# tvlabs/edge264

Measured on AMD Instinct MI355X. Metric: 1080p frames/s/GPU (bit-exact YUV) + achieved HBM GB/s vs 8 TB/s peak, higher is better.
Workload: dtype u8

## Files before the change

### edge264_amd/csrc/e264_intra.h

```cpp
#ifndef E264_INTRA_H
#define E264_INTRA_H
#include "e264_dev.h"

namespace {
#ifndef E264_HOST_INTRINSICS
E264_DEV uint32_t v_sad_u8(uint32_t a, uint32_t b, uint32_t c) { return __builtin_amdgcn_sad_u8(a, b, c); }
E264_DEV int relane(int lane) { asm volatile("" : "+v"(lane)); return lane; }
#endif

#define YT_STRIDE 32
#define YT(y, x) ytile[((y) + 1) * YT_STRIDE + (x) + 8]
#define CT_STRIDE 16
#define CT(p, y, x) ctile[p][((y) + 1) * CT_STRIDE + (x) + 4]

#define T4_STRIDE 20
struct __attribute__((aligned(16))) WaveLds {
	int16_t res[384];
	int32_t tmp[16 * T4_STRIDE];
	int32_t dc[24];
	uint8_t ytile[17 * YT_STRIDE];
	uint8_t ctile[2][9 * CT_STRIDE];
	__attribute__((aligned(4))) uint8_t fz[32];
	uint8_t pad_[8];
	__attribute__((aligned(4))) uint8_t lcol[3][16];
// ... 111 lines not shown
	int16_t *t16 = (int16_t *)L.tmp;
	if (on) {
		const int nb = __builtin_popcount(coded & 0x1111u & ((1u << (b * 4)) - 1));
		int div = qP / 6, m = qP - div * 6;
		const int shl = max(div - 6, 0), shr = max(6 - div, 0), rnd = div < 6 ? 1 << (5 - div) : 0;
		const int lo = div < 6 ? -32768 : (int)0x80000000, hi = div < 6 ? 32767 : 0x7fffffff;
		int16_t d[8];
		int lev[8];
		if (l8) {
#pragma unroll
			for (int i = 0; i < 8; i++) lev[i] = ((const int8_t *)coef_base)[nb * 64 + i * 8 + j];
		} else {
#pragma unroll
			for (int i = 0; i < 8; i++) lev[i] = ((const int16_t *)coef_base)[nb * 64 + i * 8 + j];
		}
#pragma unroll
		for (int i = 0; i < 8; i++) {
			int pos = i * 8 + j;
			int LS = wS[pos] * norm8(m, pos);
			d[i] = (int16_t)min(max((mul24(lev[i], (int)(int16_t)(LS << shl)) + rnd) >> shr, lo), hi);
		}
		idct8_1d(d);
#pragma unroll
		for (int i = 0; i < 8; i++)
			t16[b * 64 + i * 8 + j] = d[i];
	}
	wave_sync();
	if (on) {
		int i = j;
		int16_t d[8];
#pragma unroll
		for (int jj = 0; jj < 8; jj++)
			d[jj] = t16[b * 64 + i * 8 + jj];
		d[0] = (int16_t)(d[0] + 32);
		idct8_1d(d);
		int16_t *r = L.res + BYf(b * 4) * 16 + BXf(b * 4) + i;
#pragma unroll
		for (int jj = 0; jj < 8; jj++)
			r[jj * 16] = (int16_t)(d[jj] >> 6);
	}
	wave_sync();
}

E264_DEV int coef_dwords(const MbInfo &m)
{
	if (m.kind == E264_MB_ABSENT || m.kind == E264_MB_PCM || m.coded == 0)
		return 0;
	const uint32_t c = m.coded;
	int ac = __builtin_popcount(c >> 16 & 0xff) * 32;
	ac += (m.kind != E264_MB_I16x16 && (m.flags & E264_MBF_T8x8)) ? __builtin_popcount(c & 0x1111) * 128 : __builtin_popcount(c & 0xffff) * 32;
	if (m.flags & E264_MBF_LEV8) ac >>= 1;
	return (((c & E264_CODED_LUMA_DC) ? 32 : 0) + ((c & E264_CODED_CHROMA_DC) ? 16 : 0) + ac + 3) >> 2;
}
E264_DEV void coef_dma(int16_t *dst, const FrameCtx &f, const MbInfo &m, int lane)
{
	const int ndw = coef_dwords(m);
	if (ndw == 0)
		return;
	const gu32 *src = (const gu32 *)(f.payload + m.payload_off) + lane;
#ifndef E264_HOST_INTRINSICS
	typedef __attribute__((address_space(3))) void *lds_p;
	if (lane < ndw) __builtin_amdgcn_global_load_lds(src, (lds_p)dst, 4, 0, 0);
	if (ndw > 64 && 64 + lane < ndw) __builtin_amdgcn_global_load_lds(src + 64, (lds_p)(dst + 128), 4, 0, 0);
	if (ndw > 128 && 128 + lane < ndw) __builtin_amdgcn_global_load_lds(src + 128, (lds_p)(dst + 256), 4, 0, 0);
	if (ndw > 192 && 192 + lane < ndw) __builtin_amdgcn_global_load_lds(src + 192, (lds_p)(dst + 384), 4, 0, 0);
#else
	for (int k = 0; k < 4; k++)
		if (64 * k + lane < ndw) ((uint32_t *)dst)[64 * k + lane] = src[64 * k];
#endif
}
E264_DEV void coef_dma_wait()
{
#ifndef E264_HOST_INTRINSICS
	asm volatile("s_waitcnt vmcnt(0)" ::: "memory");
#endif
	wave_sync();
}
E264_DEV void slice_cache(WaveLds &L, const FrameCtx &f, int slice, int lane)
{
	if (E264_FIRST(L.ws_slice) == slice)
		return;
	cslice_t s = f.slices + slice;
	wave_sync();
	const gu32 *g4 = (const gu32 *)((const gu8 *)s + offsetof(E264SliceParams, weightScale4x4));
	const gu32 *g8 = (const gu32 *)((const gu8 *)s + offsetof(E264SliceParams, weightScale8x8));
	if (lane < 24) ((uint32_t *)L.ws)[lane] = g4[lane];
	else if (lane < 56) ((uint32_t *)L.ws)[lane] = g8[lane - 24];
	if (lane == 0) { L.ws_slice = slice; L.ws_idc = s->weighted_bipred_idc; }
	wave_sync();
}

template <int PLANES = 3>
E264_DEV void compute_residual(WaveLds &L, const int16_t *coefs, const FrameCtx &f, const MbInfo &m, bool inter, int lane)
{
	uint32_t *rz = (uint32_t *)L.res;
	rz[lane] = 0; rz[lane + 64] = 0; rz[lane + 128] = 0;
	const uint32_t coded = m.coded;
	const int16_t *pl = coefs;
	const int16_t *ldc = nullptr, *cdc = nullptr;
	if (coded & E264_CODED_LUMA_DC) { ldc = pl; pl += 16; }
	if (coded & E264_CODED_CHROMA_DC) { cdc = pl; pl += 8; }
	const uint8_t *co = (const uint8_t *)pl;
	const bool l8 = m.flags & E264_MBF_LEV8;
	const int lsz = l8 ? 1 : 2;
	const uint8_t *ws4 = L.ws, *ws8 = L.ws + 96;
	if (lane < 24) L.dc[lane] = 0;
	wave_sync();
	if (!coded) return;

	if ((PLANES & 1) && ldc && lane < 16) {
		int r = lane >> 2, l = lane & 3, acc = 0;
#pragma unroll
		for (int i = 0; i < 4; i++)
#pragma unroll
			for (int mm = 0; mm < 4; mm++) {
				int v = ldc[4 * i + mm];
				bool neg = (((0xA6C0 >> (4 * r)) >> mm) ^ ((0xA6C0 >> (4 * l)) >> i)) & 1;
				acc += neg ? -v : v;
			}
		int qP = m.qp[0];
		int LS = (ws4[0] * norm4(qP % 6, 0)) << (qP / 6);
		int k = (r >> 1) * 8 + (l >> 1) * 4 + (r & 1) * 2 + (l & 1);
		L.dc[k] = (int)((uint32_t)acc * (uint32_t)LS + 32u) >> 6;
	}
	if ((PLANES & 2) && cdc && lane >= 16 && lane < 24) {
		int n = lane & 3, pc = (lane >> 2) & 1;
		int c0 = cdc[pc], c4 = cdc[4 + pc], c2 = cdc[2 + pc], c6 = cdc[6 + pc];
		int v = n == 0 ? c0 + c4 + c2 + c6 : n == 1 ? c0 - c4 + c2 - c6 : n == 2 ? c0 + c4 - c2 - c6 : c0 - c4 - c2 + c6;
		int qP = pc ? m.qp[2] : m.qp[1];
		int LS = (ws4[(1 + pc + (inter ? 3 : 0)) * 16] * norm4(qP % 6, 0)) << (qP / 6);
		L.dc[16 + pc * 4 + n] = (int)((uint32_t)v * (uint32_t)LS) >> 5;
	}
	wave_sync();

	if (m.kind == E264_MB_I16x16) {
		if ((PLANES & 1) && (coded & (0xffff | E264_CODED_LUMA_DC)))
			idct4x4_blocks(L, 16, coded & 0xffff, true, ldc != nullptr, co, l8, ws4, m.qp[0], 0, 0, 16, lane);
		co += __builtin_popcount(coded & 0xffff) * 16 * lsz;
	} else if (m.flags & E264_MBF_T8x8) {
		if ((PLANES & 1) && (coded & 0x1111))
			idct8x8_blocks(L, coded, co, l8, ws8 + (inter ? 64 : 0), m.qp[0], lane);
		co += __builtin_popcount(coded & 0x1111) * 64 * lsz;
	} else {
		if ((PLANES & 1) && (coded & 0xffff))
			idct4x4_blocks(L, 16, coded & 0xffff, false, false, co, l8, ws4 + (inter ? 3 : 0) * 16, m.qp[0], 0, 0, 16, lane);
		co += __builtin_popcount(coded & 0xffff) * 16 * lsz;
	}
	if ((PLANES & 2) && (coded & (0xff0000 | E264_CODED_CHROMA_DC))) {
		int k = lane >> 2;
		int pc = (k >> 2) & 1;
		idct4x4_blocks(L, 8, coded >> 16 & 0xff, true, cdc != nullptr, co, l8, ws4 + (1 + pc + (inter ? 3 : 0)) * 16, pc ? m.qp[2] : m.qp[1], 16, 256, 8, lane);
	}
}

#define LP(l, m, r) (((l) + 2 * (m) + (r) + 2) >> 2)
#ifndef E264_I4_UNROLL
#define E264_I4_UNROLL 10
#endif
#include "e264_intra_tab.h"

struct IntraNb { uint32_t y, c; bool oky, okc; };
E264_DEV IntraNb issue_intra_neighbours(const FrameCtx &f, int mbx, int mby, int lane)
{
	IntraNb n;
	const bool left = lane >= 32 && lane < 48;
	const bool topY = lane < 25;
	const int x = lane - 1, gx = mbx * 16 + x;
	n.oky = topY ? (mby > 0 && gx >= 0 && gx < f.W) : (left && mbx > 0);
	const gu8 *Y = f.cur + (size_t)(mby * 16) * f.sY + mbx * 16;
	const ptrdiff_t offY = topY ? (ptrdiff_t)x - f.sY : (ptrdiff_t)(lane - 32) * f.sY - 1;
	if (n.oky) n.y = Y[offY];
	const bool topC = lane < 18;
	const int xc = lane % 9 - 1;
	const int pl = topC ? lane / 9 : (lane - 32) >> 3;
	n.okc = topC ? (mby > 0 && mbx * 8 + xc >= 0) : (left && mbx > 0);
	const gu8 *C = plane_base(f, f.cur, 1 + (pl & 1)) + (size_t)(mby * 8) * f.sC + mbx * 8;
	const ptrdiff_t offC = topC ? (ptrdiff_t)xc - f.sC : (ptrdiff_t)(lane & 7) * f.sC - 1;
	if (n.okc) n.c = C[offC];
	return n;
}
E264_DEV void commit_intra_neighbours(WaveLds &L, const IntraNb &n, int lane)
{
	const bool left = lane >= 32 && lane < 48;
	const uint8_t vy = n.oky ? (uint8_t)n.y : 0, vc = n.okc ? (uint8_t)n.c : 0;
	if (lane < 25) L.YT(-1, lane - 1) = vy;
	else if (left) { L.YT(lane - 32, -1) = vy; L.lcol[0][lane - 32] = vy; }
	if (lane < 18) L.CT(lane / 9, -1, lane % 9 - 1) = vc;
	else if (left) { L.CT((lane - 32) >> 3, lane & 7, -1) = vc; L.lcol[1 + ((lane - 32) >> 3)][lane & 7] = vc; }
	wave_sync();
}

E264_DEV int intra4x4_tab(const WaveLds &L, uint32_t e, int X0, int Y0, int mode)
{
	const uint8_t *org = &L.YT(Y0 - 1, X0 - 1);
	const bool dc = mode >= 2 && mode <= 5;
	const int a = org[e & 255], b = org[e >> 8 & 255], c = org[e >> 16 & 255];
	int vd = 128;
	if (dc) {
		const uint32_t w = *(const uint32_t *)(org + 1);
		const int st = (int)v_sad_u8(w, 0, 0);
		const int sl = org[YT_STRIDE] + org[2 * YT_STRIDE] + org[3 * YT_STRIDE] + org[4 * YT_STRIDE];
		vd = mode == 2 ? (st + sl + 4) >> 3 : mode == 3 ? (st + 2) >> 2 : mode == 4 ? (sl + 2) >> 2 : 128;
	}
	const int ty = (int)(e >> 24), sh = ty >> 3;
	const int v = (a + (ty & 3) * b + ((ty & 4) ? c : 0) + ((1 << sh) >> 1)) >> sh;
	return dc ? vd : v;
}

E264_DEV int intra4x4_px(const WaveLds &L, int X0, int Y0, int mode, int x, int y)
{
#define T(i) ((int)L.YT(Y0 - 1, X0 + (i)))
#define Lf(i) ((int)L.YT(Y0 + (i), X0 - 1))
#define TR(i) ((i) < 4 || has_tr ? T(i) : T(3))
	const bool has_tr = (mode == 6 || mode == 11);
	switch (mode) {
	default:
	case 0: return T(x);
	case 1: return Lf(y);
	case 2: return (T(0) + T(1) + T(2) + T(3) + Lf(0) + Lf(1) + Lf(2) + Lf(3) + 4) >> 3;
	case 3: return (T(0) + T(1) + T(2) + T(3) + 2) >> 2;
	case 4: return (Lf(0) + Lf(1) + Lf(2) + Lf(3) + 2) >> 2;
	case 5: return 128;
	case 6: case 7:
		return (x == 3 && y == 3) ? (TR(6) + 3 * TR(7) + 2) >> 2 : LP(TR(x + y), TR(x + y + 1), TR(x + y + 2));
	case 8:
		if (x > y) return LP(T(x - y - 2), T(x - y - 1), T(x - y));
		if (x < y) return LP(y - x - 2 < 0 ? T(-1) : Lf(y - x - 2), Lf(y - x - 1), Lf(y - x));
		return LP(T(0), T(-1), Lf(0));
	case 9: {
		int z = 2 * x - y, i = x - (y >> 1);
		if (z >= 0 && !(z & 1)) return (T(i - 1) + T(i) + 1) >> 1;
		if (z >= 0) return LP(T(i - 2), T(i - 1), T(i));
		if (z == -1) return LP(Lf(0), T(-1), T(0));
		return LP(Lf(y - 1), Lf(y - 2), y - 3 < 0 ? T(-1) : Lf(y - 3)); }
	case 10: {
		int z = 2 * y - x, i = y - (x >> 1);
#define L_(j) ((j) < 0 ? T(-1) : Lf(j))
// ... 78 lines not shown
		const int corner = T(-1);
		int Hh = 0, V = 0;
		for (int i = 0; i < 8; i++) {
			Hh += (i + 1) * (byte_of(tw, 8 + i) - (i == 7 ? corner : byte_of(tw, 6 - i)));
			V += (i + 1) * (byte_of(lw, 8 + i) - (i == 7 ? corner : byte_of(lw, 6 - i)));
		}
		int a = 16 * (byte_of(lw, 15) + byte_of(tw, 15)), b = (5 * Hh + 32) >> 6, c = (5 * V + 32) >> 6;
		for (int i = 0; i < 4; i++) out[i] = clip255((a + b * (X + i - 7) + c * (Yr - 7) + 16) >> 5);
		return; }
	}
#undef T
#undef Lf
}

E264_DEV int intra_chroma_px(const WaveLds &L, int p, int mode, int x, int y)
{
#define T(i) ((int)L.CT(p, -1, (i)))
#define Lf(i) ((int)L.CT(p, (i), -1))
	switch (mode) {
	default:
	case 0: case 1: case 2: case 3: {
		if (mode == 3) return 128;
		int bx = x >> 2, by = y >> 2;
		int t = 0, l = 0;
		t = (int)v_sad_u8(*(const uint32_t *)&L.CT(p, -1, bx * 4), 0, 0);
		l = (int)v_sad_u8(((const uint32_t *)L.lcol[1 + p])[by], 0, 0);
		if (mode == 1) return (t + 2) >> 2;
		if (mode == 2) return (l + 2) >> 2;
		if (bx == by) return (t + l + 4) >> 3;
		return bx ? (t + 2) >> 2 : (l + 2) >> 2; }
	case 4: return Lf(y);
	case 5: return T(x);
	case 6: {
		const uint32_t tw[2] = {*(const uint32_t *)&L.CT(p, -1, 0), *(const uint32_t *)&L.CT(p, -1, 4)};
		const uint32_t lw[2] = {((const uint32_t *)L.lcol[1 + p])[0], ((const uint32_t *)L.lcol[1 + p])[1]};
		const int corner = T(-1);
		int Hh = 0, V = 0;
		for (int i = 0; i < 4; i++) {
			Hh += (i + 1) * (byte_of(tw, 4 + i) - (i == 3 ? corner : byte_of(tw, 2 - i)));
			V += (i + 1) * (byte_of(lw, 4 + i) - (i == 3 ? corner : byte_of(lw, 2 - i)));
		}
		int a = 16 * (byte_of(lw, 7) + byte_of(tw, 7)), b = (34 * Hh + 32) >> 6, c = (34 * V + 32) >> 6;
		return clip255((a + b * (x - 3) + c * (y - 3) + 16) >> 5); }
	}
#undef T
#undef Lf
}

#ifndef E264_INTRA_LAUNDER
#define E264_INTRA_LAUNDER 5
#endif
template <int WHICH, int PLANES = 3>
E264_DEV void recon_mb(WaveLds &L, const FrameCtx &f, const MbInfo &m, int mbx, int mby, int lane, const uint32_t *i4tab, const int16_t *coefs,
	int16_t *coefs_next, const uint32_t *next_rec, MbInfo &mn PH_PARAMS)
{
	if (m.kind == E264_MB_ABSENT)
		return;
	const bool par = m.kind == E264_MB_INTER || m.kind == E264_MB_PCM;
	if ((WHICH == 1 && !par) || (WHICH == 2 && par))
		return;
	cslice_t s = f.slices + m.slice;
	const gu8 *pl = f.payload + m.payload_off;
	const int k = lane >> 2, r = lane & 3;
	const int X = BXf(k), Yr = BYf(k) + r;
	gu8 *dY = f.cur + (size_t)(mby * 16 + Yr) * f.sY + mbx * 16 + X;
	const int cpl = lane >> 5, cy = (lane >> 2) & 7, cx = (lane & 3) * 2;
	gu8 *dC = plane_base(f, f.cur, 1 + cpl) + (size_t)(mby * 8 + cy) * f.sC + mbx * 8 + cx;

	if (m.kind == E264_MB_PCM) {
		*(gu32 *)dY = *(const gu32 *)(pl + Yr * 16 + X);
		*(gu16 *)dC = *(const gu16 *)(pl + 256 + cpl * 64 + cy * 8 + cx);
		return;
	}
	const uint32_t modes_lo = m.modes_lo, modes_hi = m.modes_hi;
	IntraNb nbv;
	nbv.oky = nbv.okc = false;
	if (WHICH != 1 && m.kind != E264_MB_INTER)
		nbv = issue_intra_neighbours(f, mbx, mby, (E264_INTRA_LAUNDER & 2) ? relane(lane) : lane);
	PH(2);
	if (next_rec) {
		mn = mb_from_lds(next_rec);
		coef_dma(coefs_next, f, mn, lane);
	}
	slice_cache(L, f, m.slice, lane);
	PH(3);
	compute_residual<PLANES>(L, coefs, f, m, WHICH == 2 ? false : m.kind == E264_MB_INTER, (E264_INTRA_LAUNDER & 4) ? relane(lane) : lane);
	PH(4);

	int pY[4], pC[2];
	bool tile_luma = false;
	if (WHICH != 1 && m.kind != E264_MB_INTER) {
		commit_intra_neighbours(L, nbv, (E264_INTRA_LAUNDER & 8) ? relane(lane) : lane);
		PH(5);
		if (!(PLANES & 1)) {
		} else if (m.kind == E264_MB_I16x16) {
			intra16x16_pred(L, m.i16_mode, X, Yr, pY);
		} else if (m.kind == E264_MB_I4x4) {
			tile_luma = true;
			static constexpr int F4[10] = {0, 1, 4, 5, 6, 7, 12, 13, 14, 15}, S4[10] = {0, 0, 2, 3, 8, 9, 10, 11, 0, 0};
			const bool second = lane >= 16;
			const int hl16 = lane & 15, px = hl16 & 3, py = hl16 >> 2;
			auto mode_of = [&](int blk) { return (int)(((blk < 8 ? modes_lo : modes_hi) >> (4 * (blk & 7))) & 15); };
			int mode_n = second ? mode_of(S4[0]) : mode_of(F4[0]);
			uint32_t e_n = i4tab[mode_n * 16 + hl16];
#pragma unroll
			for (int t = 0; t < 10; t++) {
				const bool on = (t >= 2 && t <= 7) ? lane < 32 : lane < 16;
				const int mode = mode_n;
				const uint32_t e = e_n;
				if (t < 9) {
					mode_n = second ? mode_of(S4[t + 1]) : mode_of(F4[t + 1]);
					e_n = i4tab[mode_n * 16 + hl16];
				}
				const int X0 = second ? BXf(S4[t]) : BXf(F4[t]), Y0 = second ? BYf(S4[t]) : BYf(F4[t]);
				int v = 0;
				if (on) {
					const int rres = L.res[(Y0 + py) * 16 + X0 + px];
					v = intra4x4_tab(L, e, X0, Y0, mode);
					v = clip255(w16(v + rres));
				}
				wave_sync();
				if (on)
					L.YT(Y0 + py, X0 + px) = (uint8_t)v;
				wave_sync();
			}
		} else {
			tile_luma = true;
			const uint32_t *i8tab = i4tab + 14 * 16;
			const int l8 = (E264_INTRA_LAUNDER & 1) ? relane(lane) : lane;
			uint32_t e_n = i8tab[i8_nibble(I8_SPEC_LO, I8_SPEC_HI, (int)(modes_lo & 255)) * 64 + l8];
#pragma unroll 1
			for (int b = 0; b < 4; b++) {
				const uint32_t e = e_n;
				if (b < 3)
					e_n = i8tab[i8_nibble(I8_SPEC_LO, I8_SPEC_HI, (int)(modes_lo >> (8 * b + 8) & 255)) * 64 + l8];
				intra8x8_block(L, e, BXf(b * 4), BYf(b * 4), (int)(modes_lo >> (8 * b) & 255), l8);
			}
		}
		PH(6);
		if (PLANES & 2) {
			pC[0] = intra_chroma_px(L, cpl, m.chroma_mode, cx, cy);
			pC[1] = intra_chroma_px(L, cpl, m.chroma_mode, cx + 1, cy);
		}
	}
	if (PLANES & 1) {
		uint32_t outw;
		if (tile_luma) {
			outw = *(const uint32_t *)&L.YT(Yr, X);
		} else {
			const int16_t *rr = L.res + Yr * 16 + X;
			outw = (uint32_t)clip255(w16(pY[0] + rr[0])) | (uint32_t)clip255(w16(pY[1] + rr[1])) << 8 |
				(uint32_t)clip255(w16(pY[2] + rr[2])) << 16 | (uint32_t)clip255(w16(pY[3] + rr[3])) << 24;
		}
		PH(7);
		*(gu32 *)dY = outw;
	}
	if (PLANES & 2) {
		const int16_t *rc = L.res + 256 + cpl * 64 + cy * 8 + cx;
		*(gu16 *)dC = (uint16_t)(clip255(w16(pC[0] + rc[0])) | clip255(w16(pC[1] + rc[1])) << 8);
	}
}

#ifndef E264_INTRA_SLACK
#define E264_INTRA_SLACK 0
#endif

template <int NW>
struct __attribute__((aligned(16))) IntraLds {
	int16_t coef[NW][2][512];
	uint32_t hdrs[NW][64 * 8];
	WaveLds w[NW];
	int progress[E264_MAX_ROWS];
	int next_row;
	uint32_t i4tab[14 * 16 + 9 * 64];
};

#ifndef E264_INTRA_DYNROWS
#define E264_INTRA_DYNROWS 1
#endif
template <int NW>
E264_DEV int intra_next_row(int *next_row, int y, int lane)
{
	if (!E264_INTRA_DYNROWS || NW == 1)
		return y + NW;
	int ny = 0;
	if (lane == 0) ny = E264_ROW_TAKE(next_row);
	return E264_FIRST(ny);
}

template <int NW, int PLANES = 3>
E264_DEV void intra_kernel_body(IntraLds<NW> &S, const E264Job &job, const int tid, const bool use_bitmap = true)
{
	WaveLds *const lds = S.w;
	uint32_t (*const hdrs)[64 * 8] = S.hdrs;
	int *const progress = S.progress;
	uint32_t *const i4tab = S.i4tab;
	const int lane = tid & 63;
	const int wave = E264_FIRST(tid >> 6);
	FrameCtx f;
	if (!open_frame(f, job))
		return;
	if (f.h->n_coded_mbs == f.h->n_inter_mbs)
		return;
#if defined(E264_ABL_INTRA_STOP) && E264_ABL_INTRA_STOP == 1
	if (f.wm > 0) return;
#endif
	for (int i = tid; i < f.hm; i += NW * 64)
		progress[i] = 0;
	if (tid == 0) S.next_row = NW;
	for (int i = tid; i < 14 * 16 + 9 * 64; i += NW * 64)
		i4tab[i] = i < 14 * 16 ? c_i4tab[i] : c_i8tab[i - 14 * 16];
	E264_WG_SYNC();
#if defined(E264_ABL_INTRA_STOP) && E264_ABL_INTRA_STOP == 2
	if (f.wm > 0) return;
#endif
	WaveLds &L = lds[wave];
	if (lane == 0) L.ws_slice = -1;
	wave_sync();
	const gu8 *mbs_g = f.mbs_g;
	const gu16 *bitmap = (f.dbk && use_bitmap) ? (const gu16 *)(f.dbk + E264_BITMAP_OFF(f.wm * f.hm)) : nullptr;
	const int ntx16 = (f.wm + 15) >> 4;
	PH_DECL;
#pragma unroll 1
	for (int y = wave; y < f.hm; y = intra_next_row<NW>(&S.next_row, y, lane)) {
		bool row_start = true;
#pragma unroll 1
		for (int x0 = 0; x0 < f.wm; x0 += 64) {
			const int xl = x0 + lane;
			if (bitmap) {
				const bool mine = xl < f.wm && (bitmap[(size_t)y * ntx16 + (xl >> 4)] >> (xl & 15) & 1);
				if (E264_BALLOT(mine) == 0) {
					if (lane == 0)
						E264_PROGRESS_STORE(&progress[y], min(x0 + 64, f.wm));
					continue;
				}
			}
			v4u h0v = {0, 0, 0, 0}, h1v = {0, 0, 0, 0};
			uint32_t kup = E264_MB_ABSENT;
			if (xl < f.wm) {
				const gv4u *rp = (const gv4u *)(mbs_g + (size_t)(y * f.wm + xl) * sizeof(E264Mb));
				h0v = rp[0]; h1v = rp[1];
				if (y > 0) kup = *(const gu32 *)(mbs_g + (size_t)((y - 1) * f.wm + xl) * sizeof(E264Mb));
			}
			wave_sync();
			*(v4u *)&hdrs[wave][lane * 8] = h0v;
			*(v4u *)&hdrs[wave][lane * 8 + 4] = h1v;
			wave_sync();
			if (kup >> 8 & E264_MBF_DONE) kup = E264_MB_ABSENT;
			kup &= 255u;
			const int kind = (xl < f.wm && !(h0v.x >> 8 & E264_MBF_DONE)) ? (int)(h0v.x & 255) : E264_MB_ABSENT;
			unsigned long long todo = E264_BALLOT(kind == E264_MB_I4x4 || kind == E264_MB_I8x8 || kind == E264_MB_I16x16);
			const unsigned long long upi = E264_BALLOT(kup == E264_MB_I4x4 || kup == E264_MB_I8x8 || kup == E264_MB_I16x16);
			const int xe = min(x0 + 64, f.wm);
			const unsigned long long depmask = upi | upi << 1 | upi >> 1 | (x0 > 0 ? 1ull : 0ull) | (x0 + 64 < f.wm ? 1ull << 63 : 0ull);
			if (todo == 0 || (int)__builtin_ctzll(todo) > 0) {
				const int upto = todo ? x0 + (int)__builtin_ctzll(todo) : xe;
				if (lane == 0)
					E264_PROGRESS_STORE(&progress[y], upto);
			}
			MbInfo mi, mn;
			int buf = 0;
			if (todo) {
				mi = mb_from_lds(&hdrs[wave][__builtin_ctzll(todo) * 8]);
				coef_dma(S.coef[wave][buf], f, mi, lane);
			}
#pragma unroll 1
			while (todo) {
				const int x = x0 + (int)__builtin_ctzll(todo);
				todo &= todo - 1;
				const uint32_t *next_rec = todo ? &hdrs[wave][__builtin_ctzll(todo) * 8] : nullptr;
				PH(0);
				const bool dep = depmask >> (x - x0) & 1;
#ifdef E264_ABL_INTRA_NOWAIT
				if (false) {
#else
				if (y > 0 && dep) {
#endif
					int want = min(x + 2 + (row_start ? E264_INTRA_SLACK : 0), f.wm);
					row_start = false;
					while (lds_load_relaxed(&progress[y - 1]) < want)
						E264_SLEEP();
					E264_FENCE_ACQUIRE();
				}
				PH(1);
				coef_dma_wait();
				recon_mb<2, PLANES>(L, f, mi, x, y, lane, i4tab, S.coef[wave][buf], S.coef[wave][buf ^ 1], next_rec, mn PH_ARGS);
				PH(8);
#ifndef E264_ABL_INTRA_NOFENCE
				E264_FENCE_RELEASE();
#endif
				PH(9);
				const int upto = todo ? x0 + (int)__builtin_ctzll(todo) : xe;
				if (lane == 0)
					E264_PROGRESS_STORE(&progress[y], upto);
				if (next_rec) { mi = mn; buf ^= 1; }
			}
		}
	}
#ifdef E264_PHASE_INTRA
	PH_FLUSH_DBK(lane);
#endif
}

}
#endif
```

### edge264_amd/csrc/e264_kernels.hip

```cpp
#include <hip/hip_runtime.h>
#include <stdint.h>
#include "../../include/edge264_cmd.h"
#include "e264_kernels.h"
#include "e264_dev.h"
#include "e264_pred.h"
#include "e264_dbkp.h"
#include "e264_dbk.h"
#include "e264_intra.h"
#include "e264_expand.h"

static __device__ __forceinline__ void xcd_tile(int &bx, int &by)
{
	const unsigned gx = gridDim.x, nwg = gx * gridDim.y;
	const unsigned lin = blockIdx.y * gx + blockIdx.x;
	const unsigned q = nwg >> 3, r = nwg & 7, xcd = lin & 7;
	const unsigned v = (xcd < r ? xcd * (q + 1) : r * (q + 1) + (xcd - r) * q) + (lin >> 3);
	by = (int)(v / gx);
	bx = (int)(v - (unsigned)by * gx);
}

#ifndef E264_PRED_WAVES_PER_EU
#define E264_PRED_WAVES_PER_EU 4
#endif
__attribute__((amdgpu_waves_per_eu(E264_PRED_WAVES_PER_EU, E264_PRED_WAVES_PER_EU))) __global__ __launch_bounds__(PT_NT) void e264_pred_kernel(const E264Job *jobs, int mode)
// ... 31 lines not shown
	__shared__ IntraLds<16> S;
	if (blockIdx.y == 0) intra_kernel_body<16, 1>(S, jobs[blockIdx.x], (int)threadIdx.x, false);
	else intra_kernel_body<16, 2>(S, jobs[blockIdx.x], (int)threadIdx.x, false);
}

template <int NW> __global__ __launch_bounds__(NW * 64) void e264_deblock_kernel(const E264Job *jobs)
{
	__shared__ DkLds<NW> S;
	deblock_kernel_body<NW>(S, jobs[blockIdx.x], (int)threadIdx.x);
}
template <int NW> __global__ __launch_bounds__(NW * 64) void e264_deblock2_kernel(const E264Job *jobs)
{
	__shared__ Dk2Lds<NW> S;
	deblock2_kernel_body<NW>(S, jobs[blockIdx.x], (int)threadIdx.x);
}
template <int NW> __global__ __launch_bounds__(NW * 64) void e264_deblock2_planes_kernel(const E264Job *jobs)
{
	__shared__ DkPlanesLds<NW> S;
	deblock2_planes_kernel_body<NW>(S, jobs[blockIdx.x], blockIdx.y != 0, (int)threadIdx.x);
}

extern "C" const char *e264_kernel_build_flags(void)
{
	return ""
#if E264_DBK_GS == 2
		" E264_DBK_GS=2"
#endif
#ifdef E264_ABL_NOBH
		" E264_ABL_NOBH"
#endif
#ifdef E264_ABL_NOEDGE
		" E264_ABL_NOEDGE"
#endif
#ifdef E264_ABL_NOLOAD
		" E264_ABL_NOLOAD"
#endif
#ifdef E264_ABL_NOLUMA
		" E264_ABL_NOLUMA"
#endif
#ifdef E264_ABL_DBKP_NOMOT
		" E264_ABL_DBKP_NOMOT"
#endif
#ifdef E264_ABL_DBK_NOFILTER
		" E264_ABL_DBK_NOFILTER"
#endif
#ifdef E264_ABL_DBK_NOLOAD
		" E264_ABL_DBK_NOLOAD"
#endif
#ifdef E264_ABL_DBK_NOSTORE
		" E264_ABL_DBK_NOSTORE"
#endif
#ifdef E264_ABL_INTRA_NOWAIT
		" E264_ABL_INTRA_NOWAIT"
#endif
#ifdef E264_ABL_INTRA_STOP
		" E264_ABL_INTRA_STOP"
#endif
#ifdef E264_ABL_DBKP_STORE1
		" E264_ABL_DBKP_STORE1"
#endif
#ifdef E264_ABL_DBKP_NOPIECES
		" E264_ABL_DBKP_NOPIECES"
#endif

#ifdef E264_ABL_INTRA_NOFENCE
		" E264_ABL_INTRA_NOFENCE"
#endif
#ifdef E264_ABL_DBK_NOWAIT
		" E264_ABL_DBK_NOWAIT"
#endif
#ifdef E264_PHASE_TIMING
		" E264_PHASE_TIMING"
#endif
#ifdef E264_DBK_TIMELINE
		" E264_DBK_TIMELINE"
#endif
#ifdef E264_PHASE_INTRA
		" E264_PHASE_INTRA"
#endif
#ifdef E264_PRED_HPAIR
		" E264_PRED_HPAIR"
#endif
#ifdef E264_PRED_CHROMA_LAST
		" E264_PRED_CHROMA_LAST"
#endif
#ifdef E264_PRED_CLASS_PACKED
		" E264_PRED_CLASS_PACKED"
#endif
		;
}

__global__ __launch_bounds__(XP_NT) void e264_expand_kernel(const E264Job *jobs)
{
	expand_thread(jobs[blockIdx.y], blockIdx.x * XP_NT + threadIdx.x, gridDim.x * XP_NT);
}

extern "C" int e264_pred_tiles(int width_mbs, int height_mbs)
{
	return ((width_mbs + PT_W - 1) / PT_W) * ((height_mbs + PT_H - 1) / PT_H);
}

extern "C" hipError_t e264_launch_expand(const E264Job *jobs, int n_jobs, int max_mbs, hipStream_t stream)
{
	if (n_jobs > 0)
		hipLaunchKernelGGL(e264_expand_kernel, dim3((max_mbs + XP_NT - 1) / XP_NT, n_jobs), dim3(XP_NT), 0, stream, jobs);
	return hipGetLastError();
// ... 94 lines not shown
```

### edge264_amd/synth.py

```python
from __future__ import annotations

import numpy as np

from . import packet as P

_QPC = list(range(30)) + [29, 30, 31, 32, 32, 33, 34, 34, 35, 35, 36, 36, 37, 37, 37, 38, 38, 38, 39, 39, 39, 39]


def chroma_qp(qp: int, offset: int) -> int:
    return _QPC[min(max(qp + offset, 0), 51)]


I4_V, I4_H, I4_DC, I4_DC_A, I4_DC_B, I4_DC_AB, I4_DDL, I4_DDL_C, I4_DDR, I4_VR, I4_HD, I4_VL, I4_VL_C, I4_HU = range(14)
(I8_V, I8_V_C, I8_V_D, I8_V_CD, I8_H, I8_H_D, I8_DC, I8_DC_A, I8_DC_AC, I8_DC_AD, I8_DC_ACD, I8_DC_B, I8_DC_BD,
 I8_DC_C, I8_DC_D, I8_DC_CD, I8_DC_AB, I8_DDL, I8_DDL_C, I8_DDL_D, I8_DDL_CD, I8_DDR, I8_DDR_C, I8_VR, I8_VR_C,
 I8_HD, I8_VL, I8_VL_C, I8_VL_D, I8_VL_CD, I8_HU, I8_HU_D) = range(32)
I16_V, I16_H, I16_DC, I16_DC_A, I16_DC_B, I16_DC_AB, I16_P = range(7)
IC_DC, IC_DC_A, IC_DC_B, IC_DC_AB, IC_H, IC_V, IC_P = range(7)


def modes4x4(a: bool, b: bool, c: bool, d: bool) -> list[int]:
    out = [I4_DC if a and b else I4_DC_A if b else I4_DC_B if a else I4_DC_AB]
    if b:
        out += [I4_V, I4_DDL if c else I4_DDL_C, I4_VL if c else I4_VL_C]
# ... 38 lines not shown

def modes_chroma(a: bool, b: bool, d: bool) -> list[int]:
    out = [IC_DC if a and b else IC_DC_A if b else IC_DC_B if a else IC_DC_AB]
    if b:
        out.append(IC_V)
    if a:
        out.append(IC_H)
    if a and b and d:
        out.append(IC_P)
    return out


_CLASS_FRACS = (
    ((0, 0),),
    ((1, 0), (2, 0), (3, 0)),
    ((0, 1), (0, 2), (0, 3)),
    ((1, 1), (1, 3), (3, 1), (3, 3)),
    ((2, 1), (2, 2), (2, 3)),
    ((1, 2), (3, 2)),
)


def range_end_options(r: np.random.Generator) -> dict:
    kw = {}
    if r.random() < 0.5:
        kw["weight_denoms"] = [(int(r.integers(0, 8)), int(r.integers(0, 8))) for _ in range(int(r.integers(1, 4)))]
        if r.random() < 0.5:
            kw["weight_denoms"].append((7, 7))
    if r.random() < 0.5:
        kw.update(weight_range=(-128, 127), offset_range=(-128, 127))
    if r.random() < 0.5:
        kw["weight_pins"] = float(r.choice([0.1, 0.3, 0.6]))
    if r.random() < 0.5:
        kw["scaling_range"] = ((1, 256), (150, 256), (200, 256))[int(r.integers(0, 3))]
    if r.random() < 0.5:
        kw["level_ends"] = True
    if r.random() < 0.5:
        kw["mv_ends"] = float(r.choice([0.02, 0.1, 0.3]))
    if r.random() < 0.5:
        kw["chroma_qp_offsets"] = (int(r.choice([-12, -6, 0, 6, 12])), int(r.choice([-12, -6, 0, 6, 12])))
    return kw


class StreamSynth:

    def __init__(self, width_mbs: int, height_mbs: int, seed: int = 0, *, cabac_like: bool = True,
                 t8x8: bool = False, scaling: bool = False, weighted: int = 0, deblock: bool = True,
                 slices_per_frame: int = 1, intra_in_inter: float = 0.05, p_skip: float = 0.1,
                 residual_prob: float = 0.3, num_refs: int = 2, mv_range: int = 64, pcm_prob: float = 0.0,
                 stress: bool = False, qp_base: int = 28, i_kinds=(P.MB_I4x4, P.MB_I16x16),
                 filter_offsets=(0, 0), deblock_idc: int = 0, n_slots: int = 6,
                 weight_denoms=None, weight_range=(-32, 96), offset_range=(-20, 20), weight_pins: float = 0.0,
                 scaling_range=(8, 40), level_ends: bool = False, mv_ends: float = 0.0, chroma_qp_offsets=None,
                 place=None, partitions=None, mv_classes=None, both_lists: bool = False, coded_all: bool = False):
        self.w, self.h = width_mbs, height_mbs
        self.rng = np.random.default_rng(seed)
        self.t8x8, self.scaling, self.weighted, self.deblock = t8x8, scaling, weighted, deblock
        self.slices_per_frame = slices_per_frame
        self.intra_in_inter, self.p_skip, self.residual_prob = intra_in_inter, p_skip, residual_prob
        self.num_refs, self.mv_range, self.pcm_prob, self.stress = num_refs, mv_range, pcm_prob, stress
        self.qp_base, self.i_kinds = qp_base, tuple(i_kinds)
        self.filter_offsets, self.deblock_idc = filter_offsets, deblock_idc
        self.n_slots = n_slots
        self.frame_no = 0
        self.refs: list[int] = []
        self.cabac_like = cabac_like
        self.weight_denoms = None if weight_denoms is None else [tuple(int(x) for x in p) for p in weight_denoms]
        self.weight_range, self.offset_range, self.weight_pins = tuple(weight_range), tuple(offset_range), weight_pins
        self.scaling_range, self.level_ends, self.mv_ends = tuple(scaling_range), level_ends, mv_ends
        self.lev_mode = 0
        assert partitions in (None, "4x4") and all(0 <= c <= 5 for c in (mv_classes or ()))
        self.place, self.partitions, self.both_lists, self.coded_all = place, partitions, both_lists, coded_all
        self.mv_classes = tuple(mv_classes) if mv_classes else None
        if chroma_qp_offsets is not None:
            self.cqp_off = (int(chroma_qp_offsets[0]), int(chroma_qp_offsets[1]))
        else:
            self.cqp_off = (int(self.rng.integers(-3, 4)), int(self.rng.integers(-3, 4)))

    def _free_slot(self) -> int:
        keep = set(self.refs[:max(self.num_refs, 2)])
        for s in range(self.n_slots):
            if s not in keep:
                return s
        raise RuntimeError("DPB too small")

    def _levels(self, n: int, qp: int, maxnz: int, lowfreq: int) -> np.ndarray:
        rng = self.rng
        c = np.zeros(n, np.int16)
        N = 4 if n == 16 else 8
        if self.lev_mode:
            return self._end_levels(n, N, maxnz, lowfreq)
        if self.stress:
            lim = 2000
        else:
            lim = max(1, min(48, 4000 // (16 << (qp // 6))))
        cnt = int(rng.integers(1, maxnz + 1))
        for _ in range(cnt):
            x, y = int(rng.integers(0, lowfreq)), int(rng.integers(0, lowfreq))
            v = int(rng.integers(-lim, lim + 1))
            c[(x % N) * N + (y % N)] = v if v else 1
        return c

    _INT16_ENDS = (32767, -32768, -32767, 16000, -16000, 127, -128, 128, -129)

    def _end_levels(self, n: int, N: int, maxnz: int, lowfreq: int) -> np.ndarray:
        rng = self.rng
        c = np.zeros(n, np.int16)
        for _ in range(int(rng.integers(1, maxnz + 1))):
            x, y = int(rng.integers(0, lowfreq)), int(rng.integers(0, lowfreq))
            if self.lev_mode == 1:
                v = self._INT16_ENDS[int(rng.integers(0, len(self._INT16_ENDS)))]
            else:
                v = int(rng.choice([-128, 127, -127, 126, int(rng.integers(-128, 128))]))
            c[(x % N) * N + (y % N)] = v if v else 1
        if self.lev_mode == 2:
            c[1], c[N] = -128, 127
        return c

    def _slice_params(self, b: P.PacketBuilder, ftype: str, first_mb: int, l0: list[int], l1: list[int]):
        rng = self.rng
        kw = dict(slice_type={"I": 2, "P": 0, "B": 1}[ftype], first_mb=first_mb, cabac=int(self.cabac_like),
                  FilterOffsetA=self.filter_offsets[0], FilterOffsetB=self.filter_offsets[1],
                  disable_deblocking_filter_idc=(self.deblock_idc if self.deblock else 1))
        if self.scaling:
            kw["weightScale4x4"] = rng.integers(*self.scaling_range, (6, 16)).astype(np.uint8)
# ... 42 lines not shown
            ftype = "I"
        dst = self._free_slot()
        b = P.PacketBuilder(W, H, dst, self.frame_no)
        if ftype == "P":
            l0, l1 = self.refs[:self.num_refs], []
        elif ftype == "B":
            l0 = self.refs[1:2] + self.refs[0:1] if len(self.refs) > 1 else self.refs[:1]
            l1 = self.refs[:2]
        else:
            l0 = l1 = []
        n_mbs = W * H
        bounds = sorted({0, *[int(x) for x in rng.integers(1, n_mbs, self.slices_per_frame - 1)]}) if self.slices_per_frame > 1 else [0]
        slice_of = np.zeros(n_mbs, np.int32)
        slice_ids = []
        for si, fm in enumerate(bounds):
            slice_ids.append(self._slice_params(b, ftype, fm, l0, l1))
            slice_of[fm:] = si
        first_of = np.array(bounds)[slice_of]
        qp = self.qp_base
        for addr in range(n_mbs):
            mbx, mby = addr % W, addr // W
            fm = int(first_of[addr])
            sidx = slice_ids[int(slice_of[addr])]

            def avail(n_addr: int, ok: bool) -> bool:
                return ok and n_addr >= fm
            A = avail(addr - 1, mbx > 0)
            B = avail(addr - W, mby > 0)
            C = avail(addr - W + 1, mby > 0 and mbx < W - 1)
            D = avail(addr - W - 1, mby > 0 and mbx > 0)
            flags = 0
            if self.deblock and self.deblock_idc != 1:
                flags |= P.MBF_DEBLOCK
                if mbx > 0 and (A or self.deblock_idc == 0):
                    flags |= P.MBF_EDGE_LEFT
                if mby > 0 and (B or self.deblock_idc == 0):
                    flags |= P.MBF_EDGE_TOP
            qp = int(np.clip(qp + rng.integers(-2, 3), 10 if not self.stress else 0, 45 if not self.stress else 51))
            qps = (qp, chroma_qp(qp, self.cqp_off[0]), chroma_qp(qp, self.cqp_off[1]))
            if self.level_ends:
                self.lev_mode = int(rng.integers(0, 3))
            placed = self.place(mbx, mby, W, H) if self.place is not None and ftype != "I" else None
            if placed is None:
                inter = ftype != "I" and rng.random() >= self.intra_in_inter
                pcm = not inter and rng.random() < self.pcm_prob
            else:
                assert placed in ("intra", "inter", "pcm"), placed
                inter, pcm = placed == "inter", placed == "pcm"
            if pcm:
                b.set_mb(addr, kind=P.MB_PCM, slice_idx=sidx, qp=(0, chroma_qp(0, self.cqp_off[0]), chroma_qp(0, self.cqp_off[1])),
                         flags=flags, nz_mask=0xffff, pcm=rng.integers(0, 256, 384, dtype=np.uint8).tobytes())
                continue
            luma_blocks, chroma_blocks, luma_dc, chroma_dc = {}, {}, None, None
            full = inter and self.coded_all
            has_res = (not inter) or full or rng.random() < self.residual_prob
            kind = P.MB_INTER
            t8 = False
            kw = {}
            if inter:
                if self.partitions == "4x4":
                    t8 = False
                else:
                    t8 = self.t8x8 and (full or rng.random() < 0.5)
                kw["motion"] = self._motion(ftype, l0, l1, t8)
            else:
                kinds = list(self.i_kinds)
                kind = int(kinds[int(rng.integers(0, len(kinds)))])
                kw["chroma_mode"] = int(rng.choice(modes_chroma(A, B, D)))
                if kind == P.MB_I16x16:
                    kw["i16_mode"] = int(rng.choice(modes16x16(A, B, D)))
                elif kind == P.MB_I8x8:
                    t8 = True
                    mm = []
                    for blk in range(4):
                        bx, by = blk & 1, blk >> 1
                        a = A if bx == 0 else True
                        bb = B if by == 0 else True
                        c = (B if bx == 0 else C) if by == 0 else (bx == 0)
                        d = (D if bx == 0 else B) if by == 0 else (A if bx == 0 else True)
                        mm.append(int(rng.choice(modes8x8(a, bb, c, d))))
                    kw["modes"] = mm
                else:
                    mm = []
                    for k in range(16):
                        bx, by = int(P.BX[k]) // 4, int(P.BY[k]) // 4
                        a = A if bx == 0 else True
                        bb = B if by == 0 else True
                        if by == 0:
                            c = B if bx < 3 else C
                        elif bx == 3:
                            c = False
                        else:
                            c = P.blk_index(bx + 1, by - 1) < k
                        d = (D if bx == 0 else B) if by == 0 else (A if bx == 0 else True)
                        mm.append(int(rng.choice(modes4x4(a, bb, c, d))))
                    kw["modes"] = mm
            nz = 0
            if has_res:
                if kind == P.MB_I16x16:
                    if rng.random() < 0.8:
                        luma_dc = self._levels(16, qp, 6, 4)
                    if rng.random() < 0.5:
                        for k in range(16):
                            if rng.random() < 0.5:
                                c = self._levels(16, qp, 4, 3)
                                c[0] = 0
                                luma_blocks[k] = c
                                nz |= 1 << k
                elif t8:
                    for blk in range(4):
                        if full or rng.random() < 0.6:
                            luma_blocks[blk * 4] = self._levels(64, qp, 8, 4)
                            nz |= 0xf << (blk * 4)
                else:
                    for k in range(16):
                        if full or rng.random() < 0.5:
                            luma_blocks[k] = self._levels(16, qp, 6, 3)
                            nz |= 1 << k
                if self.lev_mode == 2 and not luma_blocks:
                    c = self._levels(16, qp, 4, 3)
                    c[0] = 0 if kind == P.MB_I16x16 else c[0]
                    luma_blocks[0] = c if not t8 else np.resize(c, 64)
                    nz |= 1 if not t8 else 0xf
                if full or rng.random() < 0.6:
                    chroma_dc = self._levels(16, qps[1], 4, 4)[:8].copy()
                    chroma_dc[0] |= 1
                    if full or rng.random() < 0.5:
                        for k in range(8):
                            if full or rng.random() < 0.5:
                                c = self._levels(16, qps[1 + (k >> 2)], 4, 3)
                                c[0] = 0
                                chroma_blocks[k] = c
            if t8:
                flags |= P.MBF_T8x8
            b.set_mb(addr, kind=kind, slice_idx=sidx, qp=qps, flags=flags, nz_mask=nz, luma_dc=luma_dc,
                     chroma_dc=chroma_dc, luma_blocks=luma_blocks, chroma_blocks=chroma_blocks, **kw)
        self.frame_no += 1
        if ftype != "B":
            self.refs.insert(0, dst)
            del self.refs[max(self.num_refs, 2):]
        return b.finish()

    def _motion(self, ftype: str, l0: list[int], l1: list[int], t8: bool) -> dict:
        rng = self.rng
        refPic = np.full(8, -1, np.int8)
        refIdx = np.full(8, -1, np.int8)
        mvs = np.zeros((2, 16, 2), np.int16)
        r = rng.random()
        if r < self.p_skip or (r < 0.5 + self.p_skip / 2):
            shape = 0
        elif r < 0.7:
            shape = 1
        else:
            shape = 2
        if self.partitions == "4x4":
            shape = 2
        big = rng.random() < 0.05
# ... 70 lines not shown
```

Baseline: 98030.

## Route intra neighbour loads through LDS DMA and use partial vmcnt waits

Measured after the change: 98930, median of 6. No clear change (+0.9%).

```diff
diff --git a/edge264_amd/csrc/e264_intra.h b/edge264_amd/csrc/e264_intra.h
--- a/edge264_amd/csrc/e264_intra.h
+++ b/edge264_amd/csrc/e264_intra.h
@@ -187,27 +187,48 @@
 	if (m.flags & E264_MBF_LEV8) ac >>= 1;
 	return (((c & E264_CODED_LUMA_DC) ? 32 : 0) + ((c & E264_CODED_CHROMA_DC) ? 16 : 0) + ac + 3) >> 2;
 }
-E264_DEV void coef_dma(int16_t *dst, const FrameCtx &f, const MbInfo &m, int lane)
+#ifndef E264_HOST_INTRINSICS
+#pragma clang diagnostic push
+#pragma clang diagnostic ignored "-Winline-asm"
+E264_DEV uint32_t lds_addr(const void *p) { return (uint32_t)(uintptr_t)(__attribute__((address_space(3))) const void *)p; }
+E264_DEV void lds_dma_b32(const gu32 *src, void *dst) { asm volatile("s_mov_b32 m0, %1\n\ts_nop 0\n\tglobal_load_lds_dword %0, off" :: "v"(src), "s"(lds_addr(dst)) : "memory", "m0"); }
+E264_DEV void lds_dma_u8(const gu8 *src, void *dst) { asm volatile("s_mov_b32 m0, %1\n\ts_nop 0\n\tglobal_load_lds_ubyte %0, off" :: "v"(src), "s"(lds_addr(dst)) : "memory", "m0"); }
+#pragma clang diagnostic pop
+#else
+#define lds_dma_b32(src, dst) (void)(((uint32_t *)(dst))[lane] = *(src))
+#define lds_dma_u8(src, dst) (void)(((uint32_t *)(dst))[lane] = *(src))
+#endif
+E264_DEV void lds_dma_wait_older(int newer)
+{
+#ifndef E264_HOST_INTRINSICS
+	switch (newer) {
+	case 1: asm volatile("s_waitcnt vmcnt(1)" ::: "memory"); break;
+	case 2: asm volatile("s_waitcnt vmcnt(2)" ::: "memory"); break;
+	case 3: asm volatile("s_waitcnt vmcnt(3)" ::: "memory"); break;
+	case 4: asm volatile("s_waitcnt vmcnt(4)" ::: "memory"); break;
+	default: asm volatile("s_waitcnt vmcnt(0)" ::: "memory"); break;
+	}
+#endif
+	wave_sync();
+}
+E264_DEV int coef_dma(int16_t *dst, const FrameCtx &f, const MbInfo &m, int lane)
 {
 	const int ndw = coef_dwords(m);
-	if (ndw == 0)
-		return;
 	const gu32 *src = (const gu32 *)(f.payload + m.payload_off) + lane;
+	if (lane < ndw) lds_dma_b32(src, dst);
+	if (64 + lane < ndw) lds_dma_b32(src + 64, dst + 128);
+	if (128 + lane < ndw) lds_dma_b32(src + 128, dst + 256);
+	if (192 + lane < ndw) lds_dma_b32(src + 192, dst + 384);
+	return (ndw + 63) >> 6;
+}
+template <int STORES>
+E264_DEV void coef_dma_wait(bool just_asked)
+{
 #ifndef E264_HOST_INTRINSICS
-	typedef __attribute__((address_space(3))) void *lds_p;
-	if (lane < ndw) __builtin_amdgcn_global_load_lds(src, (lds_p)dst, 4, 0, 0);
-	if (ndw > 64 && 64 + lane < ndw) __builtin_amdgcn_global_load_lds(src + 64, (lds_p)(dst + 128), 4, 0, 0);
-	if (ndw > 128 && 128 + lane < ndw) __builtin_amdgcn_global_load_lds(src + 128, (lds_p)(dst + 256), 4, 0, 0);
-	if (ndw > 192 && 192 + lane < ndw) __builtin_amdgcn_global_load_lds(src + 192, (lds_p)(dst + 384), 4, 0, 0);
-#else
-	for (int k = 0; k < 4; k++)
-		if (64 * k + lane < ndw) ((uint32_t *)dst)[64 * k + lane] = src[64 * k];
-#endif
-}
-E264_DEV void coef_dma_wait()
-{
-#ifndef E264_HOST_INTRINSICS
-	asm volatile("s_waitcnt vmcnt(0)" ::: "memory");
+	static_assert(STORES == 1 || STORES == 2, "recon_mb's sample stores");
+	if (STORES == 2) asm volatile("s_waitcnt vmcnt(2)" ::: "memory");
+	else asm volatile("s_waitcnt vmcnt(1)" ::: "memory");
+	if (just_asked) asm volatile("s_waitcnt vmcnt(0)" ::: "memory");
 #endif
 	wave_sync();
 }
@@ -294,8 +315,8 @@
 #endif
 #include "e264_intra_tab.h"
 
-struct IntraNb { uint32_t y, c; bool oky, okc; };
-E264_DEV IntraNb issue_intra_neighbours(const FrameCtx &f, int mbx, int mby, int lane)
+struct IntraNb { bool oky, okc; };
+E264_DEV IntraNb issue_intra_neighbours(uint32_t (*nbst)[64], const FrameCtx &f, int mbx, int mby, int lane)
 {
 	IntraNb n;
 	const bool left = lane >= 32 && lane < 48;
@@ -304,20 +325,21 @@
 	n.oky = topY ? (mby > 0 && gx >= 0 && gx < f.W) : (left && mbx > 0);
 	const gu8 *Y = f.cur + (size_t)(mby * 16) * f.sY + mbx * 16;
 	const ptrdiff_t offY = topY ? (ptrdiff_t)x - f.sY : (ptrdiff_t)(lane - 32) * f.sY - 1;
-	if (n.oky) n.y = Y[offY];
+	if (n.oky) lds_dma_u8(Y + offY, nbst[0]);
 	const bool topC = lane < 18;
 	const int xc = lane % 9 - 1;
 	const int pl = topC ? lane / 9 : (lane - 32) >> 3;
 	n.okc = topC ? (mby > 0 && mbx * 8 + xc >= 0) : (left && mbx > 0);
 	const gu8 *C = plane_base(f, f.cur, 1 + (pl & 1)) + (size_t)(mby * 8) * f.sC + mbx * 8;
 	const ptrdiff_t offC = topC ? (ptrdiff_t)xc - f.sC : (ptrdiff_t)(lane & 7) * f.sC - 1;
-	if (n.okc) n.c = C[offC];
+	if (n.okc) lds_dma_u8(C + offC, nbst[1]);
 	return n;
 }
-E264_DEV void commit_intra_neighbours(WaveLds &L, const IntraNb &n, int lane)
-{
+E264_DEV void commit_intra_neighbours(WaveLds &L, const uint32_t (*nbst)[64], const IntraNb &n, int newer, int lane)
+{
+	lds_dma_wait_older(newer);
 	const bool left = lane >= 32 && lane < 48;
-	const uint8_t vy = n.oky ? (uint8_t)n.y : 0, vc = n.okc ? (uint8_t)n.c : 0;
+	const uint8_t vy = n.oky ? (uint8_t)nbst[0][lane] : 0, vc = n.okc ? (uint8_t)nbst[1][lane] : 0;
 	if (lane < 25) L.YT(-1, lane - 1) = vy;
 	else if (left) { L.YT(lane - 32, -1) = vy; L.lcol[0][lane - 32] = vy; }
 	if (lane < 18) L.CT(lane / 9, -1, lane % 9 - 1) = vc;
@@ -502,7 +524,7 @@
 #endif
 template <int WHICH, int PLANES = 3>
 E264_DEV void recon_mb(WaveLds &L, const FrameCtx &f, const MbInfo &m, int mbx, int mby, int lane, const uint32_t *i4tab, const int16_t *coefs,
-	int16_t *coefs_next, const uint32_t *next_rec, MbInfo &mn PH_PARAMS)
+	int16_t *coefs_next, const uint32_t *next_rec, MbInfo &mn, uint32_t (*nbst)[64] PH_PARAMS)
 {
 	if (m.kind == E264_MB_ABSENT)
 		return;
@@ -523,16 +545,19 @@
 		return;
 	}
 	const uint32_t modes_lo = m.modes_lo, modes_hi = m.modes_hi;
+	slice_cache(L, f, m.slice, lane);
 	IntraNb nbv;
 	nbv.oky = nbv.okc = false;
 	if (WHICH != 1 && m.kind != E264_MB_INTER)
-		nbv = issue_intra_neighbours(f, mbx, mby, (E264_INTRA_LAUNDER & 2) ? relane(lane) : lane);
+		nbv = issue_intra_neighbours(nbst, f, mbx, mby, (E264_INTRA_LAUNDER & 2) ? relane(lane) : lane);
 	PH(2);
+	int n_dma = 0;
 	if (next_rec) {
 		mn = mb_from_lds(next_rec);
-		coef_dma(coefs_next, f, mn, lane);
-	}
-	slice_cache(L, f, m.slice, lane);
+#ifndef E264_ABL_INTRA_NODMA
+		n_dma = coef_dma(coefs_next, f, mn, lane);
+#endif
+	}
 	PH(3);
 	compute_residual<PLANES>(L, coefs, f, m, WHICH == 2 ? false : m.kind == E264_MB_INTER, (E264_INTRA_LAUNDER & 4) ? relane(lane) : lane);
 	PH(4);
@@ -540,7 +565,7 @@
 	int pY[4], pC[2];
 	bool tile_luma = false;
 	if (WHICH != 1 && m.kind != E264_MB_INTER) {
-		commit_intra_neighbours(L, nbv, (E264_INTRA_LAUNDER & 8) ? relane(lane) : lane);
+		commit_intra_neighbours(L, nbst, nbv, n_dma, (E264_INTRA_LAUNDER & 8) ? relane(lane) : lane);
 		PH(5);
 		if (!(PLANES & 1)) {
 		} else if (m.kind == E264_MB_I16x16) {
@@ -618,6 +643,7 @@
 template <int NW>
 struct __attribute__((aligned(16))) IntraLds {
 	int16_t coef[NW][2][512];
+	uint32_t nbst[NW][2][64];
 	uint32_t hdrs[NW][64 * 8];
 	WaveLds w[NW];
 	int progress[E264_MAX_ROWS];
@@ -710,6 +736,7 @@
 			}
 			MbInfo mi, mn;
 			int buf = 0;
+			bool just_asked = true;
 			if (todo) {
 				mi = mb_from_lds(&hdrs[wave][__builtin_ctzll(todo) * 8]);
 				coef_dma(S.coef[wave][buf], f, mi, lane);
@@ -733,8 +760,8 @@
 					E264_FENCE_ACQUIRE();
 				}
 				PH(1);
-				coef_dma_wait();
-				recon_mb<2, PLANES>(L, f, mi, x, y, lane, i4tab, S.coef[wave][buf], S.coef[wave][buf ^ 1], next_rec, mn PH_ARGS);
+				coef_dma_wait<(PLANES & 1) + (PLANES >> 1)>(just_asked);
+				recon_mb<2, PLANES>(L, f, mi, x, y, lane, i4tab, S.coef[wave][buf], S.coef[wave][buf ^ 1], next_rec, mn, S.nbst[wave] PH_ARGS);
 				PH(8);
 #ifndef E264_ABL_INTRA_NOFENCE
 				E264_FENCE_RELEASE();
@@ -744,6 +771,7 @@
 				if (lane == 0)
 					E264_PROGRESS_STORE(&progress[y], upto);
 				if (next_rec) { mi = mn; buf ^= 1; }
+				just_asked = false;
 			}
 		}
 	}
diff --git a/edge264_amd/csrc/e264_kernels.hip b/edge264_amd/csrc/e264_kernels.hip
--- a/edge264_amd/csrc/e264_kernels.hip
+++ b/edge264_amd/csrc/e264_kernels.hip
@@ -107,6 +107,9 @@
 #endif
 #ifdef E264_ABL_INTRA_NOWAIT
 		" E264_ABL_INTRA_NOWAIT"
+#endif
+#ifdef E264_ABL_INTRA_NODMA
+		" E264_ABL_INTRA_NODMA"
 #endif
 #ifdef E264_ABL_INTRA_STOP
 		" E264_ABL_INTRA_STOP"
diff --git a/edge264_amd/synth.py b/edge264_amd/synth.py
--- a/edge264_amd/synth.py
+++ b/edge264_amd/synth.py
@@ -114,7 +114,7 @@
                  filter_offsets=(0, 0), deblock_idc: int = 0, n_slots: int = 6,
                  weight_denoms=None, weight_range=(-32, 96), offset_range=(-20, 20), weight_pins: float = 0.0,
                  scaling_range=(8, 40), level_ends: bool = False, mv_ends: float = 0.0, chroma_qp_offsets=None,
-                 place=None, partitions=None, mv_classes=None, both_lists: bool = False, coded_all: bool = False):
+                 place=None, partitions=None, mv_classes=None, both_lists: bool = False, coded_all: bool = False, intra_full: float = 0.0):
         self.w, self.h = width_mbs, height_mbs
         self.rng = np.random.default_rng(seed)
         self.t8x8, self.scaling, self.weighted, self.deblock = t8x8, scaling, weighted, deblock
@@ -133,6 +133,7 @@
         self.lev_mode = 0
         assert partitions in (None, "4x4") and all(0 <= c <= 5 for c in (mv_classes or ()))
         self.place, self.partitions, self.both_lists, self.coded_all = place, partitions, both_lists, coded_all
+        self.intra_full = intra_full
         self.mv_classes = tuple(mv_classes) if mv_classes else None
         if chroma_qp_offsets is not None:
             self.cqp_off = (int(chroma_qp_offsets[0]), int(chroma_qp_offsets[1]))
@@ -281,7 +282,7 @@
                          flags=flags, nz_mask=0xffff, pcm=rng.integers(0, 256, 384, dtype=np.uint8).tobytes())
                 continue
             luma_blocks, chroma_blocks, luma_dc, chroma_dc = {}, {}, None, None
-            full = inter and self.coded_all
+            full = (inter and self.coded_all) or (not inter and self.intra_full > 0 and rng.random() < self.intra_full)
             has_res = (not inter) or full or rng.random() < self.residual_prob
             kind = P.MB_INTER
             t8 = False
@@ -327,11 +328,11 @@
             nz = 0
             if has_res:
                 if kind == P.MB_I16x16:
-                    if rng.random() < 0.8:
+                    if full or rng.random() < 0.8:
                         luma_dc = self._levels(16, qp, 6, 4)
-                    if rng.random() < 0.5:
+                    if full or rng.random() < 0.5:
                         for k in range(16):
-                            if rng.random() < 0.5:
+                            if full or rng.random() < 0.5:
                                 c = self._levels(16, qp, 4, 3)
                                 c[0] = 0
                                 luma_blocks[k] = c
```
